# gwlucastrig/gridfour

Hardware: NVIDIA B200
Metric: GVRS tile decode GB/s of raw samples (config 3 shard, 180x240 tiles) (higher is better)
Workload: dtype int32

## Files before the change

### gridfour_b200/csrc/g4_canon_fast.cuh

```cuda
#pragma once
#include "g4_canon.cuh"

namespace g4 {

constexpr int kFastStageWords = 7168;
constexpr int kFastMaxSub = 1280;
#ifndef G4_FAST_SUBBITS
#define G4_FAST_SUBBITS 160
#endif
#ifndef G4_FAST_LOOKBACK
#define G4_FAST_LOOKBACK 48
#endif
constexpr uint32_t kFastSubBits = G4_FAST_SUBBITS;
constexpr uint32_t kFastLookback = G4_FAST_LOOKBACK;
constexpr int kFastLutBits = 11;
constexpr uint32_t kFastSpecial = 0x8000u;

struct CanonFastShared {
  uint32_t mlut[1 << kFastLutBits];
  uint16_t lut[1 << kFastLutBits];
  uint16_t sorted[kCanonSymbols];
  uint16_t firstCode[17], count[17], offset[17];
  uint8_t lens[kCanonSymbols + 4];
  uint16_t ctLut[256];
// ... 66 lines not shown
    while (k < 20) {
      if (pos + 5 > src.nBits) { S.error = 1; return; }
      int index = int(src.bits(pos, 5));
      pos += 5;
      int n = 1, val = index;
      if (index <= 15) prior = index;
      else if (index == 16) { n = int(src.bits(pos, 2)) + 3; pos += 2; val = prior; }
      else if (index == 17) { n = int(src.bits(pos, 3)) + 3; pos += 3; val = 0; prior = 0; }
      else if (index == 18) { n = int(src.bits(pos, 7)) + 11; pos += 7; val = 0; prior = 0; }
      else continue;
      if (k + n > 20) { S.error = 1; return; }
      for (int i = 0; i < n; i++) ctLens[k++] = uint8_t(val);
    }
  }
  uint16_t fc[17], cn[17], of[17], so[20];
  if (!canon_build_tables(ctLens, 20, fc, cn, of, so)) { S.error = 1; return; }
  int minLen = 1;
  while (minLen < 15 && cn[minLen] == 0) minLen++;
  for (int i = 0; i < 256; i++) S.ctLut[i] = 0;
  for (int l = 1; l <= 8; l++)
    for (int d = 0; d < cn[l]; d++) {
      uint32_t rev = __brev(uint32_t(fc[l] + d)) >> (32 - l);
      uint16_t entry = uint16_t(so[of[l] + d] | (l << 8));
      for (uint32_t hi = 0; hi < (1u << (8 - l)); hi++) S.ctLut[rev | (hi << l)] = entry;
    }
  int prior = 0;
  for (int i = 0; i < kCanonSymbols; i++) S.lens[i] = 0;
  for (int i = 0; i < kCanonSymbols; i++) {
    if (pos >= src.nBits) { S.error = 1; return; }
    int test;
    uint32_t e = S.ctLut[src.peek32(pos) & 0xffu];
    if (e) { test = int(e & 0xffu); pos += e >> 8; }
    else test = canon_slow_symbol(fc, cn, of, so, src, &pos, minLen > 9 ? minLen : 9);
    if (test < 0) { S.error = 1; return; }
    if (test <= 15) { S.lens[i] = uint8_t(test); prior = test; }
    else {
      int n, val = 0;
      if (test == 16) { n = int(src.bits(pos, 2)) + 3; pos += 2; val = prior; }
      else if (test == 17) { n = int(src.bits(pos, 3)) + 3; pos += 3; prior = 0; }
      else if (test == 18) { n = int(src.bits(pos, 7)) + 11; pos += 7; prior = 0; }
      else continue;
      if (i + n > kCanonSymbols) { S.error = 1; return; }
      for (int j = 0; j < n; j++) S.lens[i + j] = uint8_t(val);
      i += n - 1;
    }
  }
  if (!canon_build_tables(S.lens, kCanonSymbols, S.firstCode, S.count, S.offset, S.sorted)) { S.error = 1; return; }
  if (S.lens[kSymEot] == 0) { S.error = 1; return; }
  S.textStart = pos;
}

__device__ __forceinline__ int canon_fast_rare_symbol(const CanonFastShared& S, uint32_t e, uint32_t p0, uint32_t nBits, uint32_t* after) {
  if (e) {
    *after = p0 + ((e >> 9) & 15u);
    return int(e & 0x1ffu);
  }
  SmemBitSrc src{S.sw, nBits};
  uint32_t p = p0;
  int sym = canon_slow_symbol(S.firstCode, S.count, S.offset, S.sorted, src, &p, kFastLutBits + 1);
  *after = p;
  return sym;
}

__device__ __forceinline__ void canon_fast_count(const CanonFastShared& S, uint32_t nBits, uint32_t start, uint32_t limit,
                                                 uint32_t* endOut, uint32_t* cntOut, int* flagOut) {
  BitCursor cur;
  cur.init(S, start, limit);
  uint32_t c = 0, end;
  int flag = 0;
  for (;;) {
    if (cur.rem >= kFastLutBits) {
      const uint32_t m = S.mlut[cur.peek() & ((1u << kFastLutBits) - 1u)];
      if (m >> 28) {
        cur.skip(S, (m >> 24) & 15u);
        c += m >> 28;
        continue;
      }
    }
    const uint32_t e = S.lut[cur.peek() & ((1u << kFastLutBits) - 1u)];
    if (e - 1u < 0x7fffu) {
      if (cur.rem <= 0) { end = cur.pos(limit); break; }
      cur.skip(S, e >> 9);
      c++;
      continue;
    }
    const uint32_t p0 = cur.pos(limit);
    uint32_t after;
    const int sym = canon_fast_rare_symbol(S, e, p0, nBits, &after);
    if (sym < 0) { flag = 2; end = p0; break; }
    if (sym == kSymEsc2 || sym == kSymEsc8) {
      after += sym == kSymEsc2 ? 2u : 8u;
      if (after > nBits) { flag = 2; end = p0; break; }
    } else {
      if (p0 >= limit) { end = p0; break; }
      if (sym == kSymEot) { flag = 1; end = after; break; }
      c++;
    }
    cur.init(S, after, limit);
  }
  *endOut = end;
  *cntOut = c;
  *flagOut = flag;
}

template <int NT = kThreads>
__device__ inline void canon_fast_tables_cta(CanonFastShared& S) {
  __shared__ uint32_t cnt32[17];
  const int tid = threadIdx.x;
  if (tid < 17) cnt32[tid] = 0;
  __syncthreads();
  for (int i = tid; i < kCanonSymbols; i += NT) {
    int l = S.lens[i];
    if (l > 15) S.error = 1;
    else if (l) atomicAdd(&cnt32[l], 1u);
  }
  __syncthreads();
  if (tid == 0) {
    uint32_t code = 0, off = 0;
    S.count[0] = 0; S.firstCode[0] = 0; S.offset[0] = 0;
    S.count[16] = 0; S.firstCode[16] = 0; S.offset[16] = 0;
    for (int l = 1; l <= 15; l++) {
      uint32_t c = cnt32[l];
      S.firstCode[l] = uint16_t(code);
      S.offset[l] = uint16_t(off);
      S.count[l] = uint16_t(c);
      if (code + c > (1u << l)) S.error = 1;
      code = (code + c) << 1;
      off += c;
    }
    if (off == 0 || S.lens[kSymEot] == 0) S.error = 1;
  }
  __syncthreads();
  if (tid < 32) {
    __shared__ uint32_t nextSlot[17];
    if (tid < 17) nextSlot[tid] = S.offset[tid];
    __syncwarp();
    for (int i0 = 0; i0 < kCanonSymbols; i0 += 32) {
      const int i = i0 + tid;
      int l = i < kCanonSymbols ? S.lens[i] : 0;
      if (l > 15) l = 0;
      const uint32_t same = __match_any_sync(0xffffffffu, l);
      const uint32_t before = same & ((1u << tid) - 1u);
      if (l) S.sorted[nextSlot[l] + __popc(before)] = uint16_t(i);
      __syncwarp();
      if (l && before == 0u) nextSlot[l] += __popc(same);
      __syncwarp();
    }
  }
  __syncthreads();
}

template <int NT = kThreads>
__device__ inline void canon_fast_build_lut(CanonFastShared& S) {
  for (int e = threadIdx.x; e < (1 << kFastLutBits); e += NT) {
    uint32_t v = __brev(uint32_t(e));
    uint16_t entry = 0;
    for (int len = 1; len <= kFastLutBits; len++) {
      uint32_t code = v >> (32 - len);
      uint32_t d = code - S.firstCode[len];
      if (d < S.count[len]) {
        uint32_t sym = S.sorted[S.offset[len] + d];
        entry = uint16_t(sym | (uint32_t(len) << 9) | (sym >= 256 ? kFastSpecial : 0u));
        break;
      }
    }
    S.lut[e] = entry;
  }
  __syncthreads();
  for (int e = threadIdx.x; e < (1 << kFastLutBits); e += NT) {
    uint32_t used = 0, n = 0, syms = 0;
    while (n < 3) {
      const uint32_t x = S.lut[(uint32_t(e) >> used) & ((1u << kFastLutBits) - 1u)];
      const uint32_t len = x >> 9;
      if (x - 1u >= 0x7fffu || used + len > uint32_t(kFastLutBits)) break;
      syms |= (x & 0xffu) << (8 * n);
      used += len;
      n++;
    }
    S.mlut[e] = syms | (used << 24) | (n << 28);
  }
  __syncthreads();
}

template <class Sink, int NT = kThreads, uint32_t SUBBITS = kFastSubBits>
__device__ bool canon_fast_decode_text(CanonFastShared& S, uint32_t nBits, const uint32_t T0, uint32_t maxValues, uint32_t hintBits,
                                       Sink sink, uint32_t* endBit, uint32_t* nValues) {
  constexpr int kThreads = NT;
  constexpr int kFastRounds = kFastMaxSub / NT;
  const int tid = threadIdx.x;
  uint32_t regionEnd = nBits;
  if (hintBits && T0 + hintBits < regionEnd) regionEnd = T0 + hintBits;
  for (;;) {
    const uint32_t avail = regionEnd - T0;
    uint32_t rounds = (avail / SUBBITS + kThreads - 1) / kThreads;
    if (rounds < 1u) rounds = 1u;
    if (rounds > uint32_t(kFastRounds)) rounds = kFastRounds;
    uint32_t B = (avail + rounds * kThreads - 1) / (rounds * kThreads);
    if (B < 96u) B = 96u;
    const int nSub = int((avail + B - 1) / B);
#pragma unroll 1
    for (int i = tid; i < nSub; i += kThreads) {
      uint32_t limit = T0 + uint32_t(i + 1) * B;
      if (limit > regionEnd) limit = regionEnd;
      uint32_t from = T0 + uint32_t(i) * B;
      if (i > 0 && limit - from > kFastLookback) from = limit - kFastLookback;
      uint32_t e, c;
      int f;
      canon_fast_count(S, nBits, from, limit, &e, &c, &f);
      S.endpos[i] = e;
      S.cnt[i] = uint16_t(c);
      S.eot[i] = uint8_t(f);
      S.startv[i] = i > 0 ? 0xffffffffu : T0;
    }
    volatile uint32_t* vend = S.endpos;
    __syncthreads();
    for (int pass = 0; pass <= nSub; pass++) {
      bool any = false;
#pragma unroll 1
      for (int i = tid; i < nSub; i += kThreads) {
        if (i == 0) continue;
        const uint32_t ns = vend[i - 1];
        if (ns != S.startv[i]) {
          S.startv[i] = ns;
          uint32_t limit = T0 + uint32_t(i + 1) * B;
          if (limit > regionEnd) limit = regionEnd;
          uint32_t e, c;
          int f;
          canon_fast_count(S, nBits, ns, limit, &e, &c, &f);
          vend[i] = e;
          S.cnt[i] = uint16_t(c);
          S.eot[i] = uint8_t(f);
          any = true;
        }
      }
      if (!__syncthreads_or(any ? 1 : 0)) break;
    }
    __syncthreads();
    if (tid == 0) S.firstEot = nSub;
    __syncthreads();
#pragma unroll 1
    for (int i = tid; i < nSub; i += kThreads)
      if (S.eot[i]) atomicMin(&S.firstEot, i);
    __syncthreads();
    const int fe = S.firstEot;
    if (fe < nSub && S.eot[fe] == 2) return false;
    if (fe == nSub) {
      if (regionEnd >= nBits) return false;
      uint32_t grown = (regionEnd - T0) * 4u;
      regionEnd = (grown > nBits - T0) ? nBits : T0 + grown;
      __syncthreads();
      continue;
    }
    uint32_t mySum = 0;
#pragma unroll
    for (int j = 0; j < kFastRounds; j++) {
      int i = tid * kFastRounds + j;
      mySum += (i <= fe && i < nSub) ? S.cnt[i] : 0u;
    }
    uint32_t total;
    uint32_t ex = block_exclusive_scan<NT>(mySum, S.scan, &total);
    if (total > maxValues) return false;
    if (tid == 0) S.endBit = S.endpos[fe];
    __syncthreads();
    uint32_t* offv = S.endpos;
    {
      uint32_t run = ex;
#pragma unroll
      for (int j = 0; j < kFastRounds; j++) {
        int i = tid * kFastRounds + j;
        if (i < nSub) {
          offv[i] = run;
          run += (i <= fe) ? S.cnt[i] : 0u;
        }
      }
    }
    __syncthreads();
    bool bad = false;
    const int last = fe < nSub - 1 ? fe : nSub - 1;
    const int i0 = tid * int(rounds);
    if constexpr (Sink::kPacked) {
      if (i0 <= last) {
        const int i1 = i0 + int(rounds) - 1 < last ? i0 + int(rounds) - 1 : last;
        uint32_t limit = T0 + uint32_t(i1 + 1) * B;
        if (limit > regionEnd) limit = regionEnd;
        BitCursor cur;
        cur.init(S, S.startv[i0], limit);
        sink.begin(offv[i0]);
        bool have = false;
        for (;;) {
          if (cur.rem >= kFastLutBits) {
            const uint32_t m = S.mlut[cur.peek() & ((1u << kFastLutBits) - 1u)];
            const uint32_t n = m >> 28;
            if (n) {
              cur.skip(S, (m >> 24) & 15u);
              sink.push(m & 0xffffffu, int(n));
              have = true;
              continue;
            }
          }
          const uint32_t e = S.lut[cur.peek() & ((1u << kFastLutBits) - 1u)];
          if (e - 1u < 0x7fffu) {
            if (cur.rem <= 0) break;
            cur.skip(S, e >> 9);
            sink.push(e & 0xffu, 1);
            have = true;
            continue;
          }
          const uint32_t p0 = cur.pos(limit);
          uint32_t after;
          const int sym = canon_fast_rare_symbol(S, e, p0, nBits, &after);
          if (sym < 0) { bad = true; break; }
          if (sym == kSymEsc2 || sym == kSymEsc8) {
            if (!have) { bad = true; break; }
            const int nb = sym == kSymEsc2 ? 2 : 8;
            if (after + nb > nBits) { bad = true; break; }
            SmemBitSrc src{S.sw, nBits};
            sink.amend(nb, src.bits(after, nb));
// ... 110 lines not shown
```

### gridfour_b200/csrc/g4_lsop_fast.cu

```cuda
#include <cuda.h>
#include <cstdio>
#include <type_traits>
#include "g4_kernels.h"
#include "g4_predict.cuh"
#include "g4_lsop_common.cuh"

namespace g4 {

namespace {

constexpr int kTextThreads = 512;
constexpr int kTextThreadsSmall = 256;
constexpr uint32_t kTextSmallTile = 16384;
constexpr uint32_t kTextSubBits = 320;
constexpr int kExcWords = 128;
constexpr int kExcCap = (kExcWords - 2) / 2;
constexpr uint32_t kTextLookback = 96;
constexpr int kStageWordsPerThread = 22;
constexpr int kSpillWords = 8;
constexpr int kResidGuard = 256;
constexpr float kMagicHalf = 6291456.0f;
constexpr float kMagicHalfUp = 6291456.5f;
constexpr float kMagicInt = 12582912.0f;
constexpr float kRange = 2097152.0f;
// ... 309 lines not shown
      const uint32_t m = S.mlut[cur.peek() & ((1u << kFastLutBits) - 1u)];
      const uint32_t n = m >> 28;
      if (n) {
        cur.skip(S.sw, (m >> 24) & 15u);
        c += n;
        A.append(m & 0xffffffu, (m >> 25) & 0x18u, slot, slotWords, spill);
        continue;
      }
    }
    const uint32_t e = S.lut[cur.peek() & ((1u << kFastLutBits) - 1u)];
    uint32_t byte;
    if (e - 1u < 0x7fffu) {
      if (cur.pos >= limit) { end = cur.pos; break; }
      cur.skip(S.sw, e >> 9);
      byte = e & 0xffu;
    } else {
      const uint32_t p0 = cur.pos;
      uint32_t after;
      const int sym = canon_fast_rare_symbol(S, e, p0, nBits, &after);
      if (sym < 0) { flag = 2; end = p0; break; }
      if (sym == kSymEsc2 || sym == kSymEsc8) {
        after += sym == kSymEsc2 ? 2u : 8u;
        if (after > nBits) { flag = 2; end = p0; break; }
        flag |= kSubRare;
        cur.init(S.sw, after);
        continue;
      }
      if (p0 >= limit) { end = p0; break; }
      if (sym == kSymEot) { flag |= 1; end = after; break; }
      if (sym == kSymNull) { flag |= kSubRare; byte = 0u; }
      else byte = uint32_t(sym);
      cur.init(S.sw, after);
    }
    c++;
    A.append(byte, 8u, slot, slotWords, spill);
  }
  A.finish(slot, slotWords, spill);
  if (A.w > slotWords + uint32_t(kSpillWords)) flag |= kSubOverflow;
  *endOut = end;
  *cntOut = c;
  *flagOut = flag;
}

__device__ __forceinline__ bool text_write_sub(const CanonFastShared& S, uint32_t nBits, uint32_t start, uint32_t limit, uint32_t k0,
                                            ByteTileSink& sink) {
  BitCursor cur;
  cur.init(S, start, limit);
  sink.begin(k0);
  bool have = false, ok = true;
  for (;;) {
    if (cur.rem >= kFastLutBits) {
      const uint32_t m = S.mlut[cur.peek() & ((1u << kFastLutBits) - 1u)];
      const uint32_t n = m >> 28;
      if (n) {
        cur.skip(S, (m >> 24) & 15u);
        sink.push(m & 0xffffffu, int(n));
        have = true;
        continue;
      }
    }
    const uint32_t e = S.lut[cur.peek() & ((1u << kFastLutBits) - 1u)];
    if (e - 1u < 0x7fffu) {
      if (cur.rem <= 0) break;
      cur.skip(S, e >> 9);
      sink.push(e & 0xffu, 1);
      have = true;
      continue;
    }
    const uint32_t p0 = cur.pos(limit);
    uint32_t after;
    const int sym = canon_fast_rare_symbol(S, e, p0, nBits, &after);
    if (sym < 0) { ok = false; break; }
    if (sym == kSymEsc2 || sym == kSymEsc8) {
      const int nb = sym == kSymEsc2 ? 2 : 8;
      if (!have || after + nb > nBits) { ok = false; break; }
      SmemBitSrc src{S.sw, nBits};
      sink.amend(nb, src.bits(after, nb));
      after += nb;
    } else {
      if (p0 >= limit || sym == kSymEot) break;
      if (sym == kSymNull) sink.put_rare(INT32_MIN);
      else sink.push(uint32_t(sym), 1);
      have = true;
    }
    cur.init(S, after, limit);
  }
  sink.end();
  return ok;
}

__device__ __noinline__ void text_exceptions_sub(const CanonFastShared& S, uint32_t nBits, uint32_t start, uint32_t limit, uint32_t k0,
                                                 uint8_t* tile, uint32_t* exc, int w, int logW, uint32_t P) {
  auto image_off = [&](uint32_t k) { return image_offset(uint32_t(w), logW, P, k); };
  auto add = [&](uint32_t k, int32_t v) {
    const uint32_t slot = atomicAdd(exc, 1u);
    if (slot < uint32_t(kExcCap)) {
      exc[2 + 2 * slot] = k;
      exc[3 + 2 * slot] = uint32_t(v);
    }
  };
  SmemBitSrc src{S.sw, nBits};
  uint32_t pos = start, k = k0, pk = 0;
  bool pending = false;
  int32_t pv = 0;
  for (;;) {
    const uint32_t e = S.lut[src.peek32(pos) & ((1u << kFastLutBits) - 1u)];
    int sym;
    uint32_t after;
    if (e - 1u < 0x7fffu) { sym = int(e & 0xffu); after = pos + (e >> 9); }
    else {
      sym = canon_fast_rare_symbol(S, e, pos, nBits, &after);
      if (sym < 0) break;
    }
    if (sym == kSymEsc2 || sym == kSymEsc8) {
      const int nb = sym == kSymEsc2 ? 2 : 8;
      if (after + nb > nBits || k == k0) break;
      if (!pending) {
        pk = k - 1;
        const uint32_t o = image_off(pk);
        pv = int32_t(tile[o]) - 128;
        tile[o] = 0;
        pending = true;
      }
      pv = int32_t((uint32_t(pv) << nb) | src.bits(after, nb));
      after += nb;
    } else {
      if (pending) { add(pk, pv); pending = false; }
      if (pos >= limit || sym == kSymEot) break;
      if (sym == kSymNull) add(k, INT32_MIN);
      k++;
    }
    pos = after;
  }
  if (pending) add(pk, pv);
}

template <int NT>
__device__ int lsop_text_decode(CanonFastShared& S, uint32_t nBits, const uint32_t T0, uint32_t nInterior, uint32_t imageBytes,
                                ByteTileSink sink, uint32_t* spillArea) {
  constexpr int kRounds = kFastMaxSub / NT;
  const int tid = threadIdx.x;
  const uint32_t avail = nBits - T0;
  uint32_t rounds = (avail / kTextSubBits + NT - 1) / NT;
  if (rounds < 1u) rounds = 1u;
  if (rounds > uint32_t(kRounds)) rounds = kRounds;
  uint32_t B = (avail + rounds * NT - 1) / (rounds * NT);
  if (B < 96u) B = 96u;
  const int nSub = int((avail + B - 1) / B);
  uint32_t slotWords = (imageBytes / uint32_t(nSub)) >> 2;
  if (slotWords > uint32_t(kStageWordsPerThread) / rounds) slotWords = uint32_t(kStageWordsPerThread) / rounds;
  if (uint64_t(slotWords + uint32_t(kSpillWords)) * 4u * uint64_t(nSub) * 3u < uint64_t(nInterior) * 4u) return 2;
  uint32_t* const image32 = reinterpret_cast<uint32_t*>(sink.tile);
  if (tid == 0) S.firstEot = nSub;
#pragma unroll 1
  for (int i = tid; i < nSub; i += NT) {
    uint32_t limit = T0 + uint32_t(i + 1) * B;
    if (limit > nBits) limit = nBits;
    uint32_t from = T0 + uint32_t(i) * B;
    if (limit - from > kTextLookback) from = limit - kTextLookback;
    uint32_t e, c;
    int f;
    canon_fast_count(S, nBits, from, limit, &e, &c, &f);
    S.endpos[i] = e;
    S.startv[i] = 0xffffffffu;
  }
  volatile uint32_t* vend = S.endpos;
  __syncthreads();
  for (int pass = 0; pass <= nSub; pass++) {
    bool any = false;
#pragma unroll 1
    for (int i = tid; i < nSub; i += NT) {
      const uint32_t ns = i ? vend[i - 1] : T0;
      if (ns != S.startv[i]) {
        S.startv[i] = ns;
        uint32_t limit = T0 + uint32_t(i + 1) * B;
        if (limit > nBits) limit = nBits;
        uint32_t e, c;
        int f;
        text_stage_sub(S, nBits, ns, limit, image32 + size_t(i) * slotWords, slotWords, spillArea + size_t(i) * kSpillWords, &e, &c, &f);
        vend[i] = e;
        S.cnt[i] = uint16_t(c);
        S.eot[i] = uint8_t(f);
        any = true;
      }
    }
    if (!__syncthreads_or(any ? 1 : 0)) break;
  }
#pragma unroll 1
  for (int i = tid; i < nSub; i += NT)
    if (S.eot[i] & 3) atomicMin(&S.firstEot, i);
  __syncthreads();
  const int fe = S.firstEot;
  if (fe == nSub || (S.eot[fe] & 3) == 2) return 1;
  uint32_t mySum = 0;
#pragma unroll
  for (int j = 0; j < kRounds; j++) {
    const int i = tid * kRounds + j;
    mySum += (i <= fe && i < nSub) ? S.cnt[i] : 0u;
  }
  uint32_t total;
  const uint32_t ex = block_exclusive_scan<NT>(mySum, S.scan, &total);
  if (total != nInterior) return 1;
  uint32_t* offv = S.endpos;
  {
    uint32_t run = ex;
#pragma unroll
    for (int j = 0; j < kRounds; j++) {
      const int i = tid * kRounds + j;
      if (i < nSub) {
        offv[i] = run;
        run += (i <= fe) ? S.cnt[i] : 0u;
      }
    }
  }
  uint32_t r[kStageWordsPerThread];
#pragma unroll
  for (int j = 0; j < kStageWordsPerThread; j++) r[j] = 0;
  {
    const uint32_t perSub = uint32_t(kStageWordsPerThread) / rounds;
    for (uint32_t s = 0; s < rounds; s++) {
      const int i = tid + int(s) * NT;
      if (i <= fe && !(S.eot[i] & kSubOverflow)) {
        const uint32_t* slot = image32 + size_t(i) * slotWords;
#pragma unroll
        for (int j = 0; j < kStageWordsPerThread; j++)
          if (uint32_t(j) >= s * perSub && uint32_t(j) < s * perSub + slotWords) r[j] = slot[uint32_t(j) - s * perSub];
      }
    }
  }
  __syncthreads();
  bool bad = false;
  {
    const uint32_t perSub = uint32_t(kStageWordsPerThread) / rounds;
    for (uint32_t s = 0; s < rounds; s++) {
      const int i = tid + int(s) * NT;
      if (i > fe) continue;
      const uint32_t n = S.cnt[i];
      const int flags = S.eot[i];
      uint32_t limit = T0 + uint32_t(i + 1) * B;
      if (limit > nBits) limit = nBits;
      if (flags & kSubOverflow) {
        if (!text_write_sub(S, nBits, S.startv[i], limit, offv[i], sink)) bad = true;
        continue;
      }
      if (n == 0) continue;
      sink.begin(offv[i]);
      if (rounds == 1u) {
        const int head = sink.head;
        const uint32_t sh = 8u * uint32_t(head);
        const int nD = int((n + uint32_t(head) + 3u) >> 2);
        const uint32_t* sp = spillArea + size_t(i) * kSpillWords;
        uint32_t prev = 0;
#pragma unroll
        for (int d = 0; d < kStageWordsPerThread + kSpillWords + 1; d++) {
          if (d >= nD) break;
          uint32_t cur = 0;
          if (d < kStageWordsPerThread && uint32_t(d) < slotWords) cur = r[d];
          else if (uint32_t(d) >= slotWords && uint32_t(d) - slotWords < uint32_t(kSpillWords) && 4u * uint32_t(d) < n) cur = sp[uint32_t(d) - slotWords];
          sink.put_word(__funnelshift_l(prev, cur, sh), d == 0 ? head : 0, int(n) + head - 4 * d);
          prev = cur;
        }
        if (flags & kSubRare) text_exceptions_sub(S, nBits, S.startv[i], limit, offv[i], sink.tile, sink.exc, sink.w, sink.logW, sink.P);
        continue;
      }
#pragma unroll
      for (int j = 0; j < kStageWordsPerThread; j++) {
        const uint32_t at = (uint32_t(j) - s * perSub) * 4u;
        if (uint32_t(j) >= s * perSub && uint32_t(j) < s * perSub + slotWords && at < n) {
          const uint32_t m = n - at;
          sink.push(m >= 4u ? r[j] : (r[j] & ((1u << (8 * m)) - 1u)), m >= 4u ? 4 : int(m));
        }
      }
      if (n > slotWords * 4u) {
        const uint32_t* sp = spillArea + size_t(i) * kSpillWords;
        for (uint32_t at = slotWords * 4u; at < n; at += 4u) {
          const uint32_t wv = *sp++, m = n - at;
          sink.push(m >= 4u ? wv : (wv & ((1u << (8 * m)) - 1u)), m >= 4u ? 4 : int(m));
        }
      }
      sink.end();
      if (flags & kSubRare) text_exceptions_sub(S, nBits, S.startv[i], limit, offv[i], sink.tile, sink.exc, sink.w, sink.logW, sink.P);
    }
  }
  return __syncthreads_or(bad ? 1 : 0) ? 1 : 0;
}

template <int NT>
__global__ void __launch_bounds__(NT, NT == 512 ? 2 : 4) lsop2_text_kernel(LsopFastArgs A, uint32_t stageWords, int listBegin, int listEnd) {
  extern __shared__ __align__(128) unsigned char textSmem[];
  CanonFastShared& F = *reinterpret_cast<CanonFastShared*>(textSmem);
  uint8_t* tileImg = textSmem + text_fast_bytes(stageWords);
  __shared__ int sTile[2];
  __shared__ __align__(8) uint64_t sBar;
  const DecodeArgs& a = A.a;
  const int tid = threadIdx.x;
  const uint32_t bar = smem_u32(&sBar);
  if (tid == 0) {
    mbar_init(bar, 1);
    asm volatile("fence.mbarrier_init.release.cluster;");
    sTile[0] = listBegin + atomicAdd(a.counter, 1);
  }
  __syncthreads();
  uint32_t parity = 0;
  for (int phase = 0;; phase ^= 1) {
    const int li = sTile[phase];
    if (li >= listEnd || li >= *a.listCount) break;
    if (tid == 0) sTile[phase ^ 1] = listBegin + atomicAdd(a.counter, 1);
    const int tIdx = a.list[li];
    const uint8_t* m = A.meta + size_t(tIdx) * kLsopMetaBytes;
    const uint32_t T0 = *reinterpret_cast<const uint32_t*>(m);
    if (T0 == 0) { __syncthreads(); continue; }
    const uint8_t* packing = a.arena + a.offsets[tIdx];
    const uint32_t len = a.lens[tIdx];
    const uint32_t delta = uint32_t(reinterpret_cast<uintptr_t>(packing) & 15u);
    const uint8_t* src16 = packing - delta;
    const uint32_t span = len + delta, nBulk = span & ~15u;
    if (tid == 0 && nBulk) {
      mbar_expect_tx(bar, nBulk);
      asm volatile("cp.async.bulk.shared::cluster.global.mbarrier::complete_tx::bytes [%0], [%1], %2, [%3];" ::"r"(smem_u32(F.sw)), "l"(src16),
                   "r"(nBulk), "r"(bar)
                   : "memory");
    }
    if (tid < 64) {
      const uint32_t i = nBulk + uint32_t(tid);
      reinterpret_cast<uint8_t*>(F.sw)[i] = i < span ? src16[i] : uint8_t(0);
    }
    for (int i = tid; i < kCanonSymbols; i += NT) F.sorted[i] = reinterpret_cast<const uint16_t*>(m + kLsopMetaSorted)[i];
    if (tid < 17) {
      F.firstCode[tid] = reinterpret_cast<const uint16_t*>(m + kLsopMetaFirst)[tid];
      F.count[tid] = reinterpret_cast<const uint16_t*>(m + kLsopMetaCount)[tid];
      F.offset[tid] = reinterpret_cast<const uint16_t*>(m + kLsopMetaOffset)[tid];
    }
    if (tid == 0) F.error = 0;
    __syncthreads();
    bool ok = true;
    canon_fast_build_lut<NT>(F);
    if (nBulk) mbar_wait(bar, parity);
    parity ^= nBulk ? 1u : 0u;
    __syncthreads();
    int rc = ok ? 0 : 1;
    if (ok) {
      const uint32_t nInterior = uint32_t(A.g.R - 2) * uint32_t(A.g.C - 4);
      ByteTileSink sink;
      sink.init(tileImg, A.exc + size_t(tIdx) * kExcWords, A.g);
      if (tid == 0) asm volatile("cp.async.bulk.wait_group.read 0;" ::: "memory");
      rc = lsop_text_decode<NT>(F, span * 8u, T0 + 8u * delta, nInterior, uint32_t(A.g.tileBytes), sink,
                                reinterpret_cast<uint32_t*>(A.textStage) + size_t(blockIdx.x) * (kFastMaxSub * kSpillWords));
      if (rc == 2) {
        uint32_t endBit = 0, nv = 0;
        rc = (canon_fast_decode_text<ByteTileSink, NT, kTextSubBits>(F, span * 8u, T0 + 8u * delta, nInterior, 0u, sink, &endBit, &nv) &&
              nv == nInterior) ? 0 : 1;
      }
      ok = rc == 0;
    }
    __syncthreads();
    if (tid == 0) {
      if (rc == 1) a.status[tIdx] = G4_ERR_FORMAT;
      else if (A.exc[size_t(tIdx) * kExcWords] > uint32_t(kExcCap)) {
        A.exc[size_t(tIdx) * kExcWords] = uint32_t(kExcCap) + 1u;
        A.defer[atomicAdd(A.deferCount, 1)] = tIdx;
      }
      else {
        asm volatile("fence.proxy.async.shared::cta;" ::: "memory");
        uint8_t* dst = A.resid + kResidGuard + size_t(tIdx) * size_t(A.g.tilePitch);
        asm volatile("cp.async.bulk.global.shared::cta.bulk_group [%0], [%1], %2;" ::"l"(dst), "r"(smem_u32(tileImg)), "r"(uint32_t(A.g.tileBytes))
                     : "memory");
        asm volatile("cp.async.bulk.commit_group;" ::: "memory");
      }
    }
  }
  if (tid == 0) asm volatile("cp.async.bulk.wait_group 0;" ::: "memory");
}

#ifndef G4_WAVE_CTAS
#define G4_WAVE_CTAS 2
#endif
#ifndef G4_WAVE_WARPS
#define G4_WAVE_WARPS 8
#endif
constexpr int kWaveWarps = G4_WAVE_WARPS;
constexpr int kWaveChunkBytes = 4096;

__device__ __noinline__ int32_t wave_exception(const uint32_t* exc, int k) {
  const int n = int(exc[0]);
  for (int i = 0; i < n; i++)
    if (int(exc[2 + 2 * i]) == k) return int32_t(exc[3 + 2 * i]);
  return -128;
}

__device__ __forceinline__ int wave_rowbuf_floats(int C) { return (C + 4 + 3) & ~3; }

template <int W, bool WIDE, bool PAIR>
__global__ void __launch_bounds__(32 * kWaveWarps, G4_WAVE_CTAS) lsop3_wave_kernel(LsopFastArgs A, int* tileCounter, int listBegin, int listEnd) {
  extern __shared__ __align__(128) unsigned char waveSmem[];
  constexpr int CR = 128 / W;
  constexpr int NW = W / 4;
  constexpr int E = W - 4;
  constexpr int TPW = PAIR ? 2 : 1;
  constexpr int HL = 32 / TPW;
  constexpr uint32_t kHalfStage = uint32_t(kWaveChunkBytes) / 2;
  constexpr bool kEarlyLo = W == 16;
  const DecodeArgs& a = A.a;
  const int lane = threadIdx.x & 31, warp = threadIdx.x >> 5;
  const int half = PAIR ? lane >> 4 : 0, ks = PAIR ? lane & 15 : lane;
  const LsopFastGeom& G = A.g;
  const int R = G.R, C = G.C, nS = G.nStrips, P = G.P;
  const int rbFloats = wave_rowbuf_floats(C);
  unsigned char* ring = waveSmem + size_t(warp) * (2 * kWaveChunkBytes);
  const uint32_t rowbuf = smem_u32(waveSmem + size_t(kWaveWarps) * (2 * kWaveChunkBytes)) + uint32_t(warp * TPW + half) * uint32_t(2 * rbFloats) * 4u;
  uint64_t* bars = reinterpret_cast<uint64_t*>(waveSmem + size_t(kWaveWarps) * (2 * kWaveChunkBytes) +
                                               size_t(kWaveWarps * TPW) * (2 * rbFloats) * sizeof(float)) + 2 * warp;
  const uint32_t bar0 = smem_u32(bars);
  const uint32_t ringLane = smem_u32(ring) + uint32_t(half) * kHalfStage + uint32_t(ks * W);
  const bool isFirst = ks == 0, isLast = ks == nS - 1;
  if (lane == 0) {
    mbar_init(bar0, 1);
    mbar_init(bar0 + 8, 1);
    asm volatile("fence.mbarrier_init.release.cluster;");
  }
  __syncwarp();
  uint32_t gchunk = 0;
  for (;;) {
  int li = 0;
  if (lane == 0) li = listBegin + atomicAdd(tileCounter, TPW);
  li = __shfl_sync(0xffffffffu, li, 0);
  if (li >= listEnd || li >= *a.listCount) break;
  li += half;
  int tIdx = 0, nExc = 0;
  bool live = false;
  if (!PAIR || (li < listEnd && li < *a.listCount)) {
    tIdx = a.list[li];
    if (a.status[tIdx] == G4_OK && *reinterpret_cast<const uint32_t*>(A.meta + size_t(tIdx) * kLsopMetaBytes) != 0u) {
      nExc = int(A.exc[size_t(tIdx) * kExcWords]);
      live = nExc <= kExcCap;
    }
  }
  const uint32_t liveMask = __ballot_sync(0xffffffffu, live);
  if (liveMask == 0u) continue;
  const bool anyExc = PAIR ? __any_sync(0xffffffffu, live && nExc > 0) : nExc > 0;
  const bool active = live && ks < nS;
  const TileView t = tile_view(a.band, a.grid, tIdx);
  const uint32_t chunkBytes = uint32_t(CR * P);
  const int nChunks = G.nChunks;
  auto issue = [&](int chunk) {
    const uint32_t g = gchunk + uint32_t(chunk);
    const uint32_t bar = bar0 + 8u * (g & 1u), dst = ringLane + uint32_t(kWaveChunkBytes) * (g & 1u);
    const size_t off = size_t(chunk) * chunkBytes + kResidGuard;
    if constexpr (PAIR) {
      const int t1 = __shfl_sync(0xffffffffu, tIdx, 16);
      const uint32_t lm = __ballot_sync(0xffffffffu, live);
      if (lane == 0) {
        const bool l0 = (lm & 1u) != 0u, l1 = (lm >> 16) != 0u;
        mbar_expect_tx(bar, chunkBytes * uint32_t(int(l0) + int(l1)));
        if (l0)
          asm volatile("cp.async.bulk.shared::cluster.global.mbarrier::complete_tx::bytes [%0], [%1], %2, [%3];" ::"r"(dst),
                       "l"(A.resid + size_t(tIdx) * size_t(G.tilePitch) + off), "r"(chunkBytes), "r"(bar)
                       : "memory");
        if (l1)
          asm volatile("cp.async.bulk.shared::cluster.global.mbarrier::complete_tx::bytes [%0], [%1], %2, [%3];" ::"r"(dst + kHalfStage),
                       "l"(A.resid + size_t(t1) * size_t(G.tilePitch) + off), "r"(chunkBytes), "r"(bar)
                       : "memory");
      }
    } else if (lane == 0) {
      mbar_expect_tx(bar, chunkBytes);
      asm volatile("cp.async.bulk.shared::cluster.global.mbarrier::complete_tx::bytes [%0], [%1], %2, [%3];" ::"r"(dst),
                   "l"(A.resid + size_t(tIdx) * size_t(G.tilePitch) + off), "r"(chunkBytes), "r"(bar)
                   : "memory");
    }
  };
  issue(0);

  float u[12];
#pragma unroll
  for (int i = 0; i < 12; i++) u[i] = active ? A.coef[size_t(tIdx) * 12 + i] : 0.f;
  if (live)
    for (int c = ks; c < rbFloats; c += HL) {
      const float x = c < C ? float(t.row(0)[c]) : 0.f, y = c < C ? float(t.row(1)[c]) : 0.f;
      asm volatile("st.shared.f32 [%0], %1;" ::"r"(rowbuf + 4u * uint32_t(c)), "f"(x) : "memory");
      asm volatile("st.shared.f32 [%0], %1;" ::"r"(rowbuf + 4u * uint32_t(rbFloats + c)), "f"(y) : "memory");
    }
  const int2* side = reinterpret_cast<const int2*>(A.side + size_t(tIdx) * R) + (isLast ? 1 : 0);
  const bool needSide = active && (isFirst || isLast);
  uint32_t rr = active ? uint32_t(-ks) : 0x40000000u;
  const uint32_t nRowsIn = uint32_t(R - 2);
  int2 sideCur = make_int2(0, 0), sideNext = make_int2(0, 0);
  if (needSide && rr < nRowsIn) sideNext = side[2 * (2 + rr)];
  const int2* sideAt = side + 2 * (3 - ks);
  char* rowp = reinterpret_cast<char*>(t.base + int64_t(2 - ks) * t.pitch + ks * W);
  const int64_t rowStep = int64_t(t.pitch) * 4;
  uint32_t ringAt = ringLane;
  const uint32_t rb0 = rowbuf + uint32_t(ks * W) * 4u, rb1 = rb0 + uint32_t(rbFloats) * 4u;
  const int wInterior = C - 4;
  uint32_t badBits = 0;
  float a0[W + 4], a1[W + 4], a2[W + 4];
#pragma unroll
  for (int i = 0; i < W + 4; i++) { a0[i] = 0.f; a1[i] = 0.f; a2[i] = 0.f; }
  int32_t pa = 0, pb = 0;
  __syncwarp();

  auto step = [&](float (&am2)[W + 4], float (&am1)[W + 4], float (&cur)[W + 4], const int s) {
    if ((s & (CR - 1)) == 0) {
      const int chunk = s / CR;
      if (chunk < nChunks) {
        if (chunk + 1 < nChunks) issue(chunk + 1);
        const uint32_t g = gchunk + uint32_t(chunk);
        mbar_wait(bar0 + 8u * (g & 1u), (g >> 1) & 1u);
      }
      ringAt = ringLane + uint32_t(kWaveChunkBytes) * ((gchunk + uint32_t(chunk)) & 1u);
    }
    const bool valid = rr < nRowsIn;
    const bool first = rr == 0u;
    if (s < nS) {
     if (first) {
#pragma unroll
      for (int i = 0; i < W + 4; i += 4) {
        float4 x, y;
        asm volatile("ld.shared.v4.f32 {%0, %1, %2, %3}, [%4];" : "=f"(x.x), "=f"(x.y), "=f"(x.z), "=f"(x.w) : "r"(rb0 + 4u * i));
        asm volatile("ld.shared.v4.f32 {%0, %1, %2, %3}, [%4];" : "=f"(y.x), "=f"(y.y), "=f"(y.z), "=f"(y.w) : "r"(rb1 + 4u * i));
        am2[i] = x.x; am2[i + 1] = x.y; am2[i + 2] = x.z; am2[i + 3] = x.w;
        am1[i] = y.x; am1[i + 1] = y.y; am1[i + 2] = y.z; am1[i + 3] = y.w;
      }
     }
// ... 239 lines not shown
```

Baseline: 915.9.

## Prefetch next tile's decode tables during decode, branchless LUT build, fused first pass

The text kernel now loads the next tile's canonical-code tables and record (T0, length, offset) one word per thread while the current tile decodes, then stores them into shared memory after decoding. This removes the serialized global-load phase at the start of each tile. The LUT build replaces its per-entry search over code lengths with a branchless compare against precomputed per-length thresholds. The first sub-block pass now finds each start position with a short lookback count and stages the sub-block immediately, instead of only counting end positions. That could reduce the number of fix-up passes, but it does more work up front and the prefetch adds register and sync-ordering complexity.

New measurement: 934.4, median of 6. +2.0%, better.

```diff
diff --git a/gridfour_b200/csrc/g4_canon_fast.cuh b/gridfour_b200/csrc/g4_canon_fast.cuh
--- a/gridfour_b200/csrc/g4_canon_fast.cuh
+++ b/gridfour_b200/csrc/g4_canon_fast.cuh
@@ -242,17 +242,19 @@
 
 template <int NT = kThreads>
 __device__ inline void canon_fast_build_lut(CanonFastShared& S) {
+  uint32_t lo[kFastLutBits + 1];
+#pragma unroll
+  for (int L = 2; L <= kFastLutBits; L++) lo[L] = uint32_t(S.firstCode[L]) << (kFastLutBits - L);
+  const uint32_t hi = uint32_t(S.firstCode[kFastLutBits]) + S.count[kFastLutBits];
   for (int e = threadIdx.x; e < (1 << kFastLutBits); e += NT) {
-    uint32_t v = __brev(uint32_t(e));
+    const uint32_t u = __brev(uint32_t(e)) >> (32 - kFastLutBits);
+    uint32_t len = 1;
+#pragma unroll
+    for (int L = 2; L <= kFastLutBits; L++) len += lo[L] <= u ? 1u : 0u;
     uint16_t entry = 0;
-    for (int len = 1; len <= kFastLutBits; len++) {
-      uint32_t code = v >> (32 - len);
-      uint32_t d = code - S.firstCode[len];
-      if (d < S.count[len]) {
-        uint32_t sym = S.sorted[S.offset[len] + d];
-        entry = uint16_t(sym | (uint32_t(len) << 9) | (sym >= 256 ? kFastSpecial : 0u));
-        break;
-      }
+    if (u < hi) {
+      const uint32_t sym = S.sorted[S.offset[len] + (u >> (kFastLutBits - len)) - S.firstCode[len]];
+      entry = uint16_t(sym | (len << 9) | (sym >= 256 ? kFastSpecial : 0u));
     }
     S.lut[e] = entry;
   }
diff --git a/gridfour_b200/csrc/g4_lsop_fast.cu b/gridfour_b200/csrc/g4_lsop_fast.cu
--- a/gridfour_b200/csrc/g4_lsop_fast.cu
+++ b/gridfour_b200/csrc/g4_lsop_fast.cu
@@ -485,19 +485,28 @@
   if (uint64_t(slotWords + uint32_t(kSpillWords)) * 4u * uint64_t(nSub) * 3u < uint64_t(nInterior) * 4u) return 2;
   uint32_t* const image32 = reinterpret_cast<uint32_t*>(sink.tile);
   if (tid == 0) S.firstEot = nSub;
+  volatile uint32_t* vend = S.endpos;
 #pragma unroll 1
   for (int i = tid; i < nSub; i += NT) {
     uint32_t limit = T0 + uint32_t(i + 1) * B;
     if (limit > nBits) limit = nBits;
-    uint32_t from = T0 + uint32_t(i) * B;
-    if (limit - from > kTextLookback) from = limit - kTextLookback;
+    uint32_t ns = T0;
+    if (i > 0) {
+      const uint32_t at = T0 + uint32_t(i) * B;
+      uint32_t from = T0 + uint32_t(i - 1) * B;
+      if (at - from > kTextLookback) from = at - kTextLookback;
+      uint32_t c;
+      int f;
+      canon_fast_count(S, nBits, from, at, &ns, &c, &f);
+    }
+    S.startv[i] = ns;
     uint32_t e, c;
     int f;
-    canon_fast_count(S, nBits, from, limit, &e, &c, &f);
-    S.endpos[i] = e;
-    S.startv[i] = 0xffffffffu;
-  }
-  volatile uint32_t* vend = S.endpos;
+    text_stage_sub(S, nBits, ns, limit, image32 + size_t(i) * slotWords, slotWords, spillArea + size_t(i) * kSpillWords, &e, &c, &f);
+    vend[i] = e;
+    S.cnt[i] = uint16_t(c);
+    S.eot[i] = uint8_t(f);
+  }
   __syncthreads();
   for (int pass = 0; pass <= nSub; pass++) {
     bool any = false;
@@ -618,61 +627,84 @@
   return __syncthreads_or(bad ? 1 : 0) ? 1 : 0;
 }
 
+constexpr int kTextTableWords = (kCanonSymbols + 3 * 17 + 1) / 2;
+static_assert(offsetof(CanonFastShared, sorted) % 4 == 0 && kLsopMetaSorted % 4 == 0, "word copy of the decoding tables");
+static_assert(offsetof(CanonFastShared, firstCode) == offsetof(CanonFastShared, sorted) + 2 * kCanonSymbols &&
+                  offsetof(CanonFastShared, count) == offsetof(CanonFastShared, firstCode) + 34 &&
+                  offsetof(CanonFastShared, offset) == offsetof(CanonFastShared, count) + 34 &&
+                  kLsopMetaFirst == kLsopMetaSorted + 2 * kCanonSymbols && kLsopMetaCount == kLsopMetaFirst + 34 &&
+                  kLsopMetaOffset == kLsopMetaCount + 34,
+              "the decoding tables lie back to back in meta and in CanonFastShared");
+static_assert(kLsopMetaSorted + 4 * kTextTableWords <= kLsopMetaBytes, "the last table word stays inside the tile's meta");
+__device__ __forceinline__ uint32_t text_setup_load(const LsopFastArgs& A, int tIdx, int tid) {
+  const uint8_t* m = A.meta + size_t(tIdx) * kLsopMetaBytes;
+  if (tid < kTextTableWords) return reinterpret_cast<const uint32_t*>(m + kLsopMetaSorted)[tid];
+  if (tid == kTextTableWords) return *reinterpret_cast<const uint32_t*>(m);
+  if (tid == kTextTableWords + 1) return A.a.lens[tIdx];
+  if (tid == kTextTableWords + 2) return uint32_t(A.a.offsets[tIdx]);
+  if (tid == kTextTableWords + 3) return uint32_t(A.a.offsets[tIdx] >> 32);
+  return 0u;
+}
+__device__ __forceinline__ void text_setup_store(CanonFastShared& F, uint32_t* rec, uint32_t w, int tid) {
+  if (tid < kTextTableWords - 1) reinterpret_cast<uint32_t*>(F.sorted)[tid] = w;
+  else if (tid == kTextTableWords - 1) F.offset[16] = uint16_t(w);
+  else if (tid < kTextTableWords + 4) rec[tid - kTextTableWords] = w;
+}
+
 template <int NT>
 __global__ void __launch_bounds__(NT, NT == 512 ? 2 : 4) lsop2_text_kernel(LsopFastArgs A, uint32_t stageWords, int listBegin, int listEnd) {
   extern __shared__ __align__(128) unsigned char textSmem[];
   CanonFastShared& F = *reinterpret_cast<CanonFastShared*>(textSmem);
   uint8_t* tileImg = textSmem + text_fast_bytes(stageWords);
-  __shared__ int sTile[2];
+  __shared__ int sNext;
+  __shared__ uint32_t sRec[4];
   __shared__ __align__(8) uint64_t sBar;
+  static_assert(NT >= kTextTableWords + 4, "one set-up word per thread");
   const DecodeArgs& a = A.a;
   const int tid = threadIdx.x;
   const uint32_t bar = smem_u32(&sBar);
+  const int listCount = *a.listCount;
+  auto tile_at = [&](int li) { return li < listEnd && li < listCount ? a.list[li] : -1; };
   if (tid == 0) {
     mbar_init(bar, 1);
     asm volatile("fence.mbarrier_init.release.cluster;");
-    sTile[0] = listBegin + atomicAdd(a.counter, 1);
-  }
+    sNext = tile_at(listBegin + atomicAdd(a.counter, 1));
+  }
+  __syncthreads();
+  int tIdx = sNext;
+  if (tIdx >= 0) text_setup_store(F, sRec, text_setup_load(A, tIdx, tid), tid);
   __syncthreads();
   uint32_t parity = 0;
-  for (int phase = 0;; phase ^= 1) {
-    const int li = sTile[phase];
-    if (li >= listEnd || li >= *a.listCount) break;
-    if (tid == 0) sTile[phase ^ 1] = listBegin + atomicAdd(a.counter, 1);
-    const int tIdx = a.list[li];
-    const uint8_t* m = A.meta + size_t(tIdx) * kLsopMetaBytes;
-    const uint32_t T0 = *reinterpret_cast<const uint32_t*>(m);
-    if (T0 == 0) { __syncthreads(); continue; }
-    const uint8_t* packing = a.arena + a.offsets[tIdx];
-    const uint32_t len = a.lens[tIdx];
+  while (tIdx >= 0) {
+    const uint32_t T0 = sRec[0], len = sRec[1];
+    const uint8_t* packing = a.arena + ((uint64_t(sRec[3]) << 32) | sRec[2]);
+    const bool live = T0 != 0;
+    int nextLi = 0;
+    if (tid == 0) nextLi = listBegin + atomicAdd(a.counter, 1);
     const uint32_t delta = uint32_t(reinterpret_cast<uintptr_t>(packing) & 15u);
     const uint8_t* src16 = packing - delta;
-    const uint32_t span = len + delta, nBulk = span & ~15u;
-    if (tid == 0 && nBulk) {
-      mbar_expect_tx(bar, nBulk);
-      asm volatile("cp.async.bulk.shared::cluster.global.mbarrier::complete_tx::bytes [%0], [%1], %2, [%3];" ::"r"(smem_u32(F.sw)), "l"(src16),
-                   "r"(nBulk), "r"(bar)
-                   : "memory");
-    }
-    if (tid < 64) {
-      const uint32_t i = nBulk + uint32_t(tid);
-      reinterpret_cast<uint8_t*>(F.sw)[i] = i < span ? src16[i] : uint8_t(0);
-    }
-    for (int i = tid; i < kCanonSymbols; i += NT) F.sorted[i] = reinterpret_cast<const uint16_t*>(m + kLsopMetaSorted)[i];
-    if (tid < 17) {
-      F.firstCode[tid] = reinterpret_cast<const uint16_t*>(m + kLsopMetaFirst)[tid];
-      F.count[tid] = reinterpret_cast<const uint16_t*>(m + kLsopMetaCount)[tid];
-      F.offset[tid] = reinterpret_cast<const uint16_t*>(m + kLsopMetaOffset)[tid];
-    }
-    if (tid == 0) F.error = 0;
-    __syncthreads();
-    bool ok = true;
-    canon_fast_build_lut<NT>(F);
+    const uint32_t span = len + delta, nBulk = live ? span & ~15u : 0u;
+    if (live) {
+      if (tid == 0 && nBulk) {
+        mbar_expect_tx(bar, nBulk);
+        asm volatile("cp.async.bulk.shared::cluster.global.mbarrier::complete_tx::bytes [%0], [%1], %2, [%3];" ::"r"(smem_u32(F.sw)), "l"(src16),
+                     "r"(nBulk), "r"(bar)
+                     : "memory");
+      }
+      if (tid < 64) {
+        const uint32_t i = nBulk + uint32_t(tid);
+        reinterpret_cast<uint8_t*>(F.sw)[i] = i < span ? src16[i] : uint8_t(0);
+      }
+      canon_fast_build_lut<NT>(F);
+    }
+    if (tid == 0) sNext = tile_at(nextLi);
     if (nBulk) mbar_wait(bar, parity);
     parity ^= nBulk ? 1u : 0u;
     __syncthreads();
-    int rc = ok ? 0 : 1;
-    if (ok) {
+    const int nIdx = sNext;
+    const uint32_t w = nIdx >= 0 ? text_setup_load(A, nIdx, tid) : 0u;
+    int rc = 0;
+    if (live) {
       const uint32_t nInterior = uint32_t(A.g.R - 2) * uint32_t(A.g.C - 4);
       ByteTileSink sink;
       sink.init(tileImg, A.exc + size_t(tIdx) * kExcWords, A.g);
@@ -684,10 +716,10 @@
         rc = (canon_fast_decode_text<ByteTileSink, NT, kTextSubBits>(F, span * 8u, T0 + 8u * delta, nInterior, 0u, sink, &endBit, &nv) &&
               nv == nInterior) ? 0 : 1;
       }
-      ok = rc == 0;
-    }
+    }
+    if (nIdx >= 0) text_setup_store(F, sRec, w, tid);
     __syncthreads();
-    if (tid == 0) {
+    if (live && tid == 0) {
       if (rc == 1) a.status[tIdx] = G4_ERR_FORMAT;
       else if (A.exc[size_t(tIdx) * kExcWords] > uint32_t(kExcCap)) {
         A.exc[size_t(tIdx) * kExcWords] = uint32_t(kExcCap) + 1u;
@@ -701,6 +733,7 @@
         asm volatile("cp.async.bulk.commit_group;" ::: "memory");
       }
     }
+    tIdx = nIdx;
   }
   if (tid == 0) asm volatile("cp.async.bulk.wait_group 0;" ::: "memory");
 }
```
